# zju3dv/OnePose_Plus_Plus

Hardware: NVIDIA H100
Metric: query images/sec (512x512, 5k 3D pts) (higher is better)
Workload: dtype fp16 hi+lo operand pairs, 3 wgmma MMAs per K-step, fp32 accumulate (fp32-grade)

## Files before the change

### onepose_plus_plus_b200/csrc/opp_common.cuh

```cuda
#pragma once

#include <cuda.h>
#include <cuda_fp16.h>
#include <cuda_runtime.h>
#include <stdint.h>
#include <stdlib.h>

namespace opp {

enum Status : int {
  OPP_OK = 0,
  OPP_ERR_INVALID = 1,
  OPP_ERR_CUDA = 2,
  OPP_ERR_UNSUPPORTED = 3
};

void set_last_error(const char* fmt, ...);

#define OPP_CHECK_CUDA(expr)                                                              \
  do {                                                                                    \
    cudaError_t _e = (expr);                                                              \
    if (_e != cudaSuccess) {                                                              \
      ::opp::set_last_error("%s:%d: %s -> %s", __FILE__, __LINE__, #expr,                 \
                            cudaGetErrorString(_e));                                      \
// ... 201 lines not shown
  return r;
}
__device__ __forceinline__ void cluster_sync_all() {
  asm volatile("barrier.cluster.arrive.aligned;" ::: "memory");
  asm volatile("barrier.cluster.wait.aligned;" ::: "memory");
}

__device__ __forceinline__ uint64_t make_kmajor_sw128_desc(uint32_t smem_addr) {
  uint64_t d = 0;
  d |= static_cast<uint64_t>((smem_addr >> 4) & 0x3FFF);
  d |= static_cast<uint64_t>(1) << 16;
  d |= static_cast<uint64_t>(1024 >> 4) << 32;
  d |= static_cast<uint64_t>(1) << 62;
  return d;
}
__device__ __forceinline__ void wgmma_fence() { asm volatile("wgmma.fence.sync.aligned;" ::: "memory"); }
__device__ __forceinline__ void wgmma_commit() { asm volatile("wgmma.commit_group.sync.aligned;" ::: "memory"); }
template <int N>
__device__ __forceinline__ void wgmma_wait() {
  asm volatile("wgmma.wait_group.sync.aligned %0;" ::"n"(N) : "memory");
}
template <int N>
__device__ __forceinline__ void wgmma_m64nNk16(float (&d)[N / 2], uint64_t a_desc, uint64_t b_desc);
#define OPP_WG_ACC8(i)                                                                              \
  "+f"(d[i]), "+f"(d[i + 1]), "+f"(d[i + 2]), "+f"(d[i + 3]), "+f"(d[i + 4]), "+f"(d[i + 5]),    \
      "+f"(d[i + 6]), "+f"(d[i + 7])
template <>
__device__ __forceinline__ void wgmma_m64nNk16<64>(float (&d)[32], uint64_t a_desc, uint64_t b_desc) {
  asm volatile(
      "{\n\t"
// ... 183 lines not shown
```

### onepose_plus_plus_b200/csrc/opp_gemm.cu

```cuda
#include <cstdarg>
#include <cstdio>
#include <cstdlib>
#include <cstring>
#include <mutex>

#include "../../include/opp_b200.h"
#include "opp_gemm.cuh"

namespace opp {

static thread_local char g_last_error[512] = "";
void set_last_error(const char* fmt, ...) {
  va_list ap;
  va_start(ap, fmt);
  vsnprintf(g_last_error, sizeof(g_last_error), fmt, ap);
  va_end(ap);
}
const char* last_error() { return g_last_error; }

typedef CUresult (*EncodeTiledFn)(CUtensorMap*, CUtensorMapDataType, cuuint32_t, void*,
                                  const cuuint64_t*, const cuuint64_t*, const cuuint32_t*,
                                  const cuuint32_t*, CUtensorMapInterleave, CUtensorMapSwizzle,
                                  CUtensorMapL2promotion, CUtensorMapFloatOOBfill);

// ... 17 lines not shown
    int dev = 0;
    if (cudaGetDevice(&dev) != cudaSuccess) return 132;
    if (cudaDeviceGetAttribute(&n, cudaDevAttrMultiProcessorCount, dev) != cudaSuccess) n = 132;
  }
  return n;
}

static int make_map(CUtensorMap* map, const void* ptr, int rank, const uint64_t* dims,
                    const uint64_t* strides_elems, const uint32_t* box) {
  EncodeTiledFn fn = get_encode_fn();
  if (!fn) {
    set_last_error("cuTensorMapEncodeTiled entry point unavailable (no CUDA driver?)");
    return OPP_ERR_CUDA;
  }
  OPP_REQUIRE((reinterpret_cast<uintptr_t>(ptr) & 15) == 0, "TMA base pointer not 16B aligned");
  cuuint64_t gdim[5], gstr[4];
  cuuint32_t bdim[5], estr[5];
  for (int i = 0; i < rank; ++i) {
    gdim[i] = dims[i];
    bdim[i] = box[i];
    estr[i] = 1;
    OPP_REQUIRE(box[i] >= 1 && box[i] <= 256, "TMA box dim %d = %u out of range", i, box[i]);
  }
  for (int i = 0; i + 1 < rank; ++i) {
    gstr[i] = strides_elems[i] * 2;
    OPP_REQUIRE((gstr[i] & 15) == 0, "TMA stride %d (%llu B) not a multiple of 16", i,
                (unsigned long long)gstr[i]);
  }
  CUresult r = fn(map, CU_TENSOR_MAP_DATA_TYPE_FLOAT16, rank, const_cast<void*>(ptr), gdim, gstr,
                  bdim, estr, CU_TENSOR_MAP_INTERLEAVE_NONE, CU_TENSOR_MAP_SWIZZLE_128B,
                  CU_TENSOR_MAP_L2_PROMOTION_L2_256B, CU_TENSOR_MAP_FLOAT_OOB_FILL_NONE);
  if (r != CUDA_SUCCESS) {
    set_last_error("cuTensorMapEncodeTiled failed with CUresult %d (rank %d dims %llu %llu %llu)",
                   (int)r, rank, (unsigned long long)dims[0], (unsigned long long)dims[1],
                   (unsigned long long)(rank > 2 ? dims[2] : 0));
    return OPP_ERR_CUDA;
  }
  return OPP_OK;
}

static int map_rows(CUtensorMap* map, const void* ptr, long long k, long long rows,
                    long long batches, long long ld, long long batch_stride, int box_rows) {
  uint64_t dims[3] = {(uint64_t)k, (uint64_t)rows, (uint64_t)batches};
  uint64_t str[2] = {(uint64_t)ld, (uint64_t)batch_stride};
  uint32_t box[3] = {(uint32_t)kBlockK, (uint32_t)box_rows, 1};
  return make_map(map, ptr, 3, dims, str, box);
}

static void log_tile_once(int a_mode, const GemmShape& s, const char* epi) {
  static int on = -1;
  if (on < 0) {
    const char* e = getenv("OPP_LOG_TILES");
    on = e ? atoi(e) : 0;
  }
  if (!on) return;
  static std::mutex mu;
  static char seen[256][128];
  static int n_seen = 0;
  char key[128];
  snprintf(key, sizeof(key), "mode %d n %d block_n %d mma_n %d k %d conv_c %d stages %d alias %d cluster %d pair %d",
           a_mode, s.n_total, s.block_n, s.mma_n, s.k_chunks * kBlockK, s.conv_c, s.stages, s.acc_alias,
           s.cluster, s.pair);
  std::lock_guard<std::mutex> lock(mu);
  if (on == 2) {
    fprintf(stderr, "opp gemm tile: %s epi %s\n", key, epi);
    return;
  }
  for (int i = 0; i < n_seen; ++i)
    if (!strcmp(seen[i], key)) return;
  if (n_seen < 256) strcpy(seen[n_seen++], key);
  fprintf(stderr, "opp gemm tile: %s\n", key);
}

template <int A_MODE, class Epi, bool DYN = false>
static int launch(const TensorMaps& maps, GemmShape s, const typename Epi::Params& ep,
                  cudaStream_t stream, const int* rows_dev = nullptr, int rows_mult = 1) {
  {
// ... 3 lines not shown
      dbg = e ? atoi(e) : 0;
    }
    s.debug_skip = dbg;
    static int cap = -1;
    if (cap < 0) {
      const char* e = getenv("OPP_STAGES");
      cap = e ? atoi(e) : 0;
    }
    OPP_REQUIRE(s.mma_n >= EpiMinMmaN<Epi>::value, "GEMM tile width %d below the epilogue's minimum %d",
                s.mma_n, EpiMinMmaN<Epi>::value);
    OPP_REQUIRE(s.mma_n > 0 && gemm_pick_stages<Epi>(s, cap),
                "GEMM tile N=%d (split %d) does not fit in shared memory", s.block_n, s.split);
  }
  const int smem = gemm_smem_bytes<Epi>(s);
  log_tile_once(A_MODE, s, Epi::kName);
  const void* kern;
  if constexpr (DYN) kern = (const void*)gemm_kernel_dyn<A_MODE, Epi>;
  else kern = (const void*)gemm_kernel<A_MODE, Epi>;
  static unsigned long long attr_done = 0;
  int dev = 0;
  OPP_CHECK_CUDA(cudaGetDevice(&dev));
  if (dev < 64 && !((attr_done >> dev) & 1ull)) {
    OPP_CHECK_CUDA(
        cudaFuncSetAttribute(kern, cudaFuncAttributeMaxDynamicSharedMemorySize, 227 * 1024));
    attr_done |= 1ull << dev;
  }
  const long long total = (long long)s.batches * s.msup * s.n_tiles;
  if (total == 0) return OPP_OK;
  const int max_clusters = num_sms() / s.cluster;
  const int n_clusters = (int)(total < max_clusters ? total : max_clusters);
  cudaLaunchConfig_t cfg = {};
  cfg.gridDim = dim3(n_clusters * s.cluster);
  cfg.blockDim = dim3(gemm_threads(Epi::kGroups));
  cfg.dynamicSmemBytes = smem;
  cfg.stream = stream;
  cudaLaunchAttribute attr[2];
  attr[0].id = cudaLaunchAttributeClusterDimension;
  attr[0].val.clusterDim.x = s.cluster;
  attr[0].val.clusterDim.y = 1;
  attr[0].val.clusterDim.z = 1;
// ... 20 lines not shown
  s.cluster = pick_cluster(s.block_n, s.m_tiles);
  s.msup = (s.m_tiles + s.cluster - 1) / s.cluster;
}

static int pick_cluster(int block_n, int m_tiles) {
  static int forced = -1;
  if (forced < 0) {
    const char* e = getenv("OPP_CLUSTER");
    forced = e ? atoi(e) : 0;
  }
  int c = forced > 1 ? forced : 2;
  while (c > 1 && (mma_width_for(block_n) % (8 * c) != 0 || m_tiles < c)) c >>= 1;
  return c;
}

static int pick_block_n(int n) {
  if (n <= 256) return (n + 15) & ~15;
  if (n % 256 == 0) return 256;
  if (n % 128 == 0) return 128;
  return 256;
}

static void split_n_for_latency(GemmShape& s) {
  static int on = -1;
  if (on < 0) {
    const char* e = getenv("OPP_NSPLIT");
    on = e ? atoi(e) : 1;
  }
  if (!on) return;
  const int max_clusters = num_sms() / s.cluster;
// ... 39 lines not shown
                      int min_mma_n = 64) {
  OPP_REQUIRE(a0 && w, "null operand");
  OPP_REQUIRE(k0 > 0 && k0 % 64 == 0 && k1 % 64 == 0, "K (%d,%d) must be multiples of 64", k0,
              k1);
  OPP_REQUIRE(n > 0 && n % n_align == 0, "N=%d must be a multiple of %d", n, n_align);
  OPP_REQUIRE(batches > 0 && rows > 0, "empty GEMM");
  const int planes = split ? 2 : 1;
  memset(&s, 0, sizeof(s));
  s.batches = batches;
  s.rows = (int)rows;
  s.m_tiles = (int)((rows + kBlockM - 1) / kBlockM);
  s.block_n = pick_block_n(n);
  OPP_REQUIRE(s.block_n % 16 == 0 && s.block_n <= 256, "bad block_n %d", s.block_n);
  s.n_tiles = (n + s.block_n - 1) / s.block_n;
  s.n_total = n;
  s.k_chunks_a0 = k0 / 64;
  s.k_chunks = (k0 + k1) / 64;
  s.b_batched = w_batched;
  s.split = split ? 1 : 0;
  s.a0_lo = k0;
  s.a1_lo = k1;
  s.b_lo = k0 + k1;
  s.a0_shared = a0_shared ? 1 : 0;
  const long long ld0 = (long long)planes * k0, ld1 = (long long)planes * k1;
  int rc = map_rows(&maps.a[0], a0, ld0, rows, a0_shared ? 1 : batches, ld0, rows * ld0, kBlockM);
  if (rc) return rc;
  if (k1 > 0) {
    OPP_REQUIRE(a1, "null second A operand");
    rc = map_rows(&maps.a[1], a1, ld1, rows, batches, ld1, rows * ld1, kBlockM);
    if (rc) return rc;
// ... 134 lines not shown
  const int out_w = (in_w + 2 * pad - ksize) / stride + 1;
  TensorMaps maps;
  GemmShape s;
  memset(&s, 0, sizeof(s));
  s.batches = batch;
  s.rows = out_h * out_w;
  s.tile_w = 16;
  s.tile_h = 8;
  s.tiles_x = (out_w + s.tile_w - 1) / s.tile_w;
  s.tiles_y = (out_h + s.tile_h - 1) / s.tile_h;
  s.m_tiles = s.tiles_x * s.tiles_y;
  s.block_n = c_out_pad;
  s.n_tiles = 1;
  s.n_total = c_out_pad;
  s.conv_c = c_in_pad;
  s.conv_cchunks = (c_in_pad + 63) / 64;
  s.k_chunks = ksize * ksize * s.conv_cchunks;
  s.conv_kw = ksize;
  s.conv_pad = pad;
  s.conv_stride = stride;
  s.out_w = out_w;
  s.out_h = out_h;
  s.split = split ? 1 : 0;
  const long long C = (long long)planes * c_in_pad;
  const __half* base = (const __half*)in;
  int rc;
  if (stride == 1) {
    uint64_t dims[5] = {(uint64_t)c_in_pad, (uint64_t)planes, (uint64_t)in_w, (uint64_t)in_h, (uint64_t)batch};
    uint64_t str[4] = {(uint64_t)c_in_pad, (uint64_t)C, (uint64_t)(in_w * C), (uint64_t)((long long)in_h * in_w * C)};
    uint32_t box[5] = {64, 1, (uint32_t)s.tile_w, (uint32_t)s.tile_h, 1};
    rc = make_map(&maps.a[0], base, 5, dims, str, box);
    if (rc) return rc;
    maps.a[1] = maps.a[2] = maps.a[3] = maps.a[0];
  } else {
    for (int py = 0; py < 2; ++py)
      for (int px = 0; px < 2; ++px) {
        uint64_t dims[5] = {(uint64_t)c_in_pad, (uint64_t)planes, (uint64_t)(in_w / 2),
                            (uint64_t)(in_h / 2), (uint64_t)batch};
        uint64_t str[4] = {(uint64_t)c_in_pad, (uint64_t)(2 * C), (uint64_t)(2LL * in_w * C),
                           (uint64_t)((long long)in_h * in_w * C)};
        uint32_t box[5] = {64, 1, (uint32_t)s.tile_w, (uint32_t)s.tile_h, 1};
        rc = make_map(&maps.a[py * 2 + px], base + ((long long)py * in_w + px) * C, 5, dims, str,
                      box);
        if (rc) return rc;
      }
  }
  const long long kplane = (long long)ksize * ksize * c_in_pad;
  s.b_lo = (int)kplane;
  const long long kt = kplane * planes;
  pick_grouping(s);
  split_n_for_latency(s);
  rc = up ? fit_tile<EpiConvUp>(s) : fit_tile<EpiConv>(s);
  if (rc) return rc;
  rc = map_rows(&maps.b, w, kt, c_out_pad, 1, kt, (long long)c_out_pad * kt, s.mma_n / s.cluster);
  if (rc) return rc;
  OPP_REQUIRE(!up || (out_h % 2 == 0 && out_w % 2 == 0 && out_h >= 4 && out_w >= 4),
              "fused upsample-add needs even output dims >= 4 (got %d x %d)", out_h, out_w);
  EpiConvParams ep{(__half*)out, (long long)c_out_pad * planes, split ? c_out_pad : 0, bias,
                     (const __half*)resid, act, slope, (__half*)tok, pe, (const __half*)up,
                     out_h / 2, out_w / 2,
                     up ? (float)(out_h / 2 - 1) / (float)(out_h - 1) : 0.f,
                     up ? (float)(out_w / 2 - 1) / (float)(out_w - 1) : 0.f};
  if (up) return launch<A_CONV, EpiConvUp>(maps, s, ep, (cudaStream_t)stream);
  return launch<A_CONV, EpiConv>(maps, s, ep, (cudaStream_t)stream);
}

int opp_conv_win_pitch(int win) {
  static int pack5 = -1;
  if (pack5 < 0) {
// ... 19 lines not shown
  TensorMaps maps;
  GemmShape s;
  memset(&s, 0, sizeof(s));
  s.batches = 1;
  const int pitch = opp_conv_win_pitch(win);
  s.tile_w = pitch;
  s.tile_h = win;
  s.tiles_x = 128 / (pitch * win);
  s.tiles_y = 1;
  s.rows = matches * pitch * win;
  s.m_tiles = (matches + s.tiles_x - 1) / s.tiles_x;
  s.block_n = c_out_pad;
  s.n_tiles = 1;
  s.n_total = c_out_pad;
  s.conv_c = c_in_pad;
  s.conv_cchunks = (c_in_pad + 63) / 64;
  s.k_chunks = 9 * s.conv_cchunks;
  s.conv_kw = 3;
  s.conv_pad = 1;
  s.conv_stride = 1;
  s.out_w = pitch;
  s.out_h = win;
  s.split = split ? 1 : 0;
  const long long C = (long long)planes * c_in_pad;
  int rc;
  {
    const uint64_t iw = j_ids ? in_w : 8, ih = j_ids ? in_h : win + 2, ib = j_ids ? batch : matches;
    uint64_t dims[5] = {(uint64_t)c_in_pad, (uint64_t)planes, iw, ih, ib};
    uint64_t str[4] = {(uint64_t)c_in_pad, (uint64_t)C, (uint64_t)(iw * C), (uint64_t)(ih * iw * C)};
    uint32_t box[5] = {64, 1, (uint32_t)pitch, (uint32_t)win, 1};
    rc = make_map(&maps.a[0], in, 5, dims, str, box);
    if (rc) return rc;
    maps.a[1] = maps.a[2] = maps.a[3] = maps.a[0];
  }
  const long long kplane = 9LL * c_in_pad;
  s.b_lo = (int)kplane;
  const long long kt = kplane * planes;
  pick_grouping(s);
  rc = fit_tile<EpiWin>(s);
  if (rc) return rc;
  rc = map_rows(&maps.b, w, kt, c_out_pad, 1, kt, (long long)c_out_pad * kt, s.mma_n / s.cluster);
  if (rc) return rc;
  EpiWin::Params ep{(__half*)out, (long long)c_out_pad * planes, split ? c_out_pad : 0, bias, act, slope,
                    b_ids, j_ids, wc, stride, org, in_h, in_w};
  if (count) return launch<A_WIN, EpiWin, true>(maps, s, ep, (cudaStream_t)stream, count, pitch * win);
  return launch<A_WIN, EpiWin>(maps, s, ep, (cudaStream_t)stream);
}

int opp_sim_lse(const void* a, const void* b, float* part_m, float* part_s, int batches, int rows,
                int cols, int k, float scale, int split, opp_stream_t stream) {
  TensorMaps maps;
  GemmShape s;
  int rc = setup_rows(maps, s, a, k, nullptr, 0, b, 1, batches, rows, cols, split, 1);
  if (rc) return rc;
  EpiLse::Params ep{part_m, part_s, scale};
  return launch<A_ROWS, EpiLse>(maps, s, ep, (cudaStream_t)stream);
// ... 72 lines not shown
```

### onepose_plus_plus_b200/csrc/opp_gemm.cuh

```cuda
#pragma once

#include <type_traits>

#include "opp_common.cuh"

#ifndef OPP_CONV_GROUPS
#define OPP_CONV_GROUPS 2
#endif

namespace opp {

constexpr int kBlockM = 128;
constexpr int kBlockK = 64;
constexpr int kABytes = kBlockM * kBlockK * 2;
constexpr int kMaxStages = 8;
constexpr int kEpiParamBytes = 4096;
constexpr int kMaxEpiWarps = 8;
constexpr int gemm_threads(int groups) { return 128 + 128 * groups; }
constexpr int kProducerRegs = 40;
constexpr int kMmaRegs = 232;
static_assert(128 * kProducerRegs + 256 * kMmaRegs <= 65536, "register file of one SM");
constexpr int kMmaWidths[] = {64, 128, 208, 256};
constexpr int mma_width_for(int block_n) {
  for (int w : kMmaWidths)
    if (w >= block_n) return w;
  return 0;
}

enum AMode : int { A_ROWS = 0, A_CONV = 1, A_WIN = 2 };

struct TensorMaps {
  CUtensorMap a[4];
  CUtensorMap b;
};

struct GemmShape {
  int batches;
  int rows;
  int m_tiles;
  int n_tiles;
  int n_total;
  int block_n;
  int mma_n;
  int k_chunks;
  int stages;
  int b_batched;
  int cluster;
  int msup;
  int pair;
  int acc_alias;
  int debug_skip;
  int split;
  int b_lo;
  int k_chunks_a0;
  int a0_lo, a1_lo;
  int a0_shared;
  int conv_cchunks;
  int conv_c;
  int conv_kw;
// ... 1184 lines not shown
}

template <int N, int KS>
__device__ __forceinline__ void mma_k_steps(float (&d)[N / 2], bool split, uint64_t a_hi, uint64_t a_lo,
                                            uint64_t b_hi, uint64_t b_lo) {
#pragma unroll
  for (int k = 0; k < KS; ++k) wgmma_m64nNk16<N>(d, a_hi + 2 * k, b_hi + 2 * k);
  if (split) {
#pragma unroll
    for (int k = 0; k < KS; ++k) wgmma_m64nNk16<N>(d, a_hi + 2 * k, b_lo + 2 * k);
#pragma unroll
    for (int k = 0; k < KS; ++k) wgmma_m64nNk16<N>(d, a_lo + 2 * k, b_hi + 2 * k);
  }
}

template <int A_MODE, class Epi>
__device__ __forceinline__ void gemm_body(const TensorMaps& maps, const GemmShape& s,
                                          const typename Epi::Params& ep) {
  static_assert(Epi::kGroups == 2, "each of the two MMA warpgroups is one epilogue group");
  extern __shared__ uint8_t smem_raw[];
  uint8_t* smem = reinterpret_cast<uint8_t*>(
      (reinterpret_cast<uintptr_t>(smem_raw) + 1023) & ~static_cast<uintptr_t>(1023));
  const int planes = s.split ? 2 : 1;
  const bool nsc = s.pair == 2;
  const int b_bytes = s.mma_n * kBlockK * 2;
  const int a_stage = kABytes * planes;
  const int b_stage = b_bytes * planes;
  const int ring = s.stages * (a_stage + b_stage);
  uint8_t* smem_a = smem;
  uint8_t* smem_b = smem + s.stages * a_stage;
  constexpr bool kAccTile = !EpiFromRegs<Epi>::value;
  uint8_t* smem_acc = s.acc_alias ? smem : smem + ring;
  float* epi_smem = reinterpret_cast<float*>(smem + ring + (kAccTile && !s.acc_alias ? gemm_acc_bytes(s.mma_n) : 0));
  uint64_t* bars = reinterpret_cast<uint64_t*>(reinterpret_cast<uint8_t*>(epi_smem) +
                                               epi_smem_bytes<Epi>());
  uint64_t* full = bars;
  uint64_t* empty = bars + kMaxStages;
  uint64_t* accfree = bars + 2 * kMaxStages;

  constexpr int kProducerWarp = 4 * Epi::kGroups;
  const int warp = threadIdx.x >> 5;
  const int lane = threadIdx.x & 31;
  const int csize = nsc ? 1 : s.cluster;
  const int prank = s.cluster > 1 ? (int)cluster_ctarank() : 0;
  const int crank = nsc ? 0 : prank;
  const int nrank = nsc ? prank : 0;
  const uint16_t cmask = (uint16_t)((1u << csize) - 1u);
  const int cluster_id = blockIdx.x / s.cluster;
  const int n_clusters = gridDim.x / s.cluster;
  const int tiles_per_batch = s.msup * s.n_tiles;
  const int total_tiles = s.batches * tiles_per_batch;

  if (warp == kProducerWarp && lane == 0) {
    tma_prefetch_desc(&maps.a[0]);
    tma_prefetch_desc(&maps.b);
  }
  if (warp == 0 && lane == 0) {
    for (int i = 0; i < s.stages; ++i) {
      mbar_init(&full[i], 1);
      mbar_init(&empty[i], 2 * csize);
    }
    mbar_init(accfree, 4 * Epi::kGroups * csize);
    if constexpr (EpiExtraSmem<Epi>::value > 0) {
      uint64_t* xbar = reinterpret_cast<uint64_t*>(reinterpret_cast<uint8_t*>(epi_smem) + epi_smem_bytes<Epi>() -
                                                   EpiExtraSmem<Epi>::value + 2 * 128 * 8);
      mbar_init(&xbar[0], Epi::kExchangeArrivals);
      mbar_init(&xbar[1], Epi::kExchangeArrivals);
    }
    fence_mbar_init();
  }
  if (s.cluster > 1) cluster_sync_all(); else __syncthreads();
  pdl_sync();

  if (warp >= kProducerWarp) {
    setmaxnreg_dec<kProducerRegs>();
    if (warp == kProducerWarp) {
      int stage = 0;
      uint32_t phase = 0;
      const bool skip_b = (s.debug_skip & 1) != 0, skip_a = (s.debug_skip & 2) != 0;
      const int a_tx = A_MODE == A_WIN ? s.tiles_x * s.tile_w * s.tile_h * (kBlockK * 2) * planes : a_stage;
      const uint32_t tx_bytes = (skip_a ? 0 : a_tx) + (skip_b ? 0 : b_stage);
      int it = 0;
      for (int t = cluster_id; t < total_tiles; t += n_clusters, ++it) {
        if (s.acc_alias && it > 0) mbar_wait(accfree, (uint32_t)((it - 1) & 1));
        const int b = t / tiles_per_batch;
        const int r = t - b * tiles_per_batch;
        const int msi = r / s.n_tiles;
        const int n_tile = nsc ? nrank : r - msi * s.n_tiles;
        const int m_tile = msi * csize + crank;
        int ox0 = 0, oy0 = 0;
        if (A_MODE == A_CONV) {
          const int ty = m_tile / s.tiles_x;
          oy0 = ty * s.tile_h;
          ox0 = (m_tile - ty * s.tiles_x) * s.tile_w;
        }
// ... 6 lines not shown
          for (int wi = 0; wi < 5; ++wi) {
            int m = m_tile * s.tiles_x + wi;
            m = m < cnt ? m : cnt - 1;
            win_z[wi] = m;
            if (ep.j_ids) {
              const int j = (int)ep.j_ids[m];
              const int cy = j / ep.wc;
              win_z[wi] = (int)ep.b_ids[m];
              win_x[wi] = ep.stride * (j - cy * ep.wc) + ep.org - s.conv_pad;
              win_y[wi] = ep.stride * cy + ep.org - s.conv_pad;
            }
          }
        }
        int cc = 0, ky = 0, kx = 0, kb_tap = 0;
        for (int chunk = 0; chunk < s.k_chunks; ++chunk) {
          mbar_wait(&empty[stage], phase ^ 1);
          uint8_t* sa = smem_a + stage * a_stage;
          uint8_t* sb = smem_b + stage * b_stage;
          int kb;
          if (A_MODE == A_ROWS) {
            const bool first = chunk < s.k_chunks_a0;
            const int kc = (first ? chunk : chunk - s.k_chunks_a0) * kBlockK;
            const CUtensorMap* am = first ? &maps.a[0] : &maps.a[1];
            const int lo = first ? s.a0_lo : s.a1_lo;
            const int ba = (first && s.a0_shared) ? 0 : b;
            kb = chunk * kBlockK;
            if (elect_one()) {
              mbar_expect_tx(&full[stage], tx_bytes);
              if (!skip_a) {
                tma_load_3d(am, &full[stage], sa, kc, m_tile * kBlockM, ba);
                if (s.split) tma_load_3d(am, &full[stage], sa + kABytes, kc + lo, m_tile * kBlockM, ba);
              }
            }
          } else if constexpr (A_MODE == A_WIN) {
            kb = kb_tap + cc * kBlockK;
            const int wbytes = s.tile_w * s.tile_h * (kBlockK * 2);
#pragma unroll
            for (int wi = 0; wi < 5; ++wi) {
              if (wi >= s.tiles_x) break;
              const int bx = win_x[wi] + kx, by = win_y[wi] + ky, bz = win_z[wi];
              if (elect_one()) {
                if (wi == 0) mbar_expect_tx(&full[stage], tx_bytes);
                if (!skip_a) {
                  tma_load_5d(&maps.a[0], &full[stage], sa + wi * wbytes, cc * kBlockK, 0, bx, by, bz);
                  if (s.split)
                    tma_load_5d(&maps.a[0], &full[stage], sa + kABytes + wi * wbytes, cc * kBlockK, 1, bx, by, bz);
                }
              }
            }
            if (++cc == s.conv_cchunks) {
              cc = 0;
              kb_tap += s.conv_c;
              if (++kx == s.conv_kw) {
                kx = 0;
                ++ky;
              }
            }
          } else {
            int dy = ky - s.conv_pad, dx = kx - s.conv_pad, mi = 0;
            if (s.conv_stride == 2) {
              const int py = dy & 1, px = dx & 1;
              dy = (dy - py) >> 1;
              dx = (dx - px) >> 1;
              mi = py * 2 + px;
            }
            kb = kb_tap + cc * kBlockK;
            if (elect_one()) {
              mbar_expect_tx(&full[stage], tx_bytes);
              if (!skip_a) {
                tma_load_5d(&maps.a[mi], &full[stage], sa, cc * kBlockK, 0, ox0 + dx, oy0 + dy, b);
                if (s.split)
                  tma_load_5d(&maps.a[mi], &full[stage], sa + kABytes, cc * kBlockK, 1, ox0 + dx, oy0 + dy, b);
              }
            }
            if (++cc == s.conv_cchunks) {
              cc = 0;
              kb_tap += s.conv_c;
              if (++kx == s.conv_kw) {
                kx = 0;
                ++ky;
              }
            }
          }
          if (!skip_b && elect_one()) {
            if (csize == 1) {
              tma_load_3d(&maps.b, &full[stage], sb, kb, nrow0, bb);
              if (s.split) tma_load_3d(&maps.b, &full[stage], sb + b_bytes, s.b_lo + kb, nrow0, bb);
            } else {
              const int slice = s.mma_n / csize;
              const int soff = crank * slice * (kBlockK * 2);
              const int nrow = nrow0 + crank * slice;
              tma_load_3d_mc(&maps.b, &full[stage], sb + soff, kb, nrow, bb, cmask);
              if (s.split)
                tma_load_3d_mc(&maps.b, &full[stage], sb + b_bytes + soff, s.b_lo + kb, nrow, bb, cmask);
            }
          }
          __syncwarp();
          if (++stage == s.stages) {
            stage = 0;
            phase ^= 1;
          }
        }
      }
    }
  } else {
    setmaxnreg_inc<kMmaRegs>();
    const int g = warp >> 2;
    const int q = warp & 3;
    EpiCtx c;
    c.etid = q * 32 + lane;
    c.q = q;
    c.a_mode = A_MODE;
    c.group = g;
    c.col_first = 32 * g;
    c.col_step = 32 * Epi::kGroups;
    c.smem = epi_smem + g * (kEpiParamBytes / 8);
    c.wstage = reinterpret_cast<uint8_t*>(epi_smem) + kEpiParamBytes + warp * EpiWarpStage<Epi>::value;
    c.extra = reinterpret_cast<uint8_t*>(epi_smem) + epi_smem_bytes<Epi>() - EpiExtraSmem<Epi>::value;
    c.smem_s = smem_u32(c.smem);
    c.wstage_s = smem_u32(c.wstage);
    const uint64_t desc_tmpl = make_kmajor_sw128_desc(0);
    const uint32_t sa0 = ((smem_u32(smem_a) >> 4) & 0x3FFF) + g * ((64 * 128) >> 4);
    const uint32_t sb0 = (smem_u32(smem_b) >> 4) & 0x3FFF;
    const uint32_t a_step = (uint32_t)a_stage >> 4, b_step = (uint32_t)b_stage >> 4;
    const uint32_t a_lo_off = kABytes >> 4, b_lo_off = (uint32_t)b_bytes >> 4;
    const bool split = s.split != 0;
    const bool is_signal = q == 0 && lane == 0;
    const uint32_t pitch = (uint32_t)(s.mma_n + kAccPad);
    const uint32_t acc_w = smem_u32(smem_acc) >> 2;
    const uint32_t r0 = 64 * g + 16 * q + (lane >> 2), c0 = 2 * (lane & 3);
    auto release = [&](int st) {
      if (is_signal) {
        if (csize == 1) mbar_arrive(&empty[st]);
        else
          for (int r = 0; r < csize; ++r) mbar_arrive_cluster(&empty[st], (uint32_t)r);
      }
    };
// ... 34 lines not shown
          int rdummy;
          if (epi_row_at(s, c, (int)r0 + 8 * h, c.sgrow[h], rdummy)) c.svalid |= 1u << h;
        }
      }
      c.acc = acc_w + (uint32_t)(q * 32 + lane) * pitch;
      Epi::prefetch(ep, s, c);

      auto mma_tile = [&](auto n_c, auto tail_c) {
        constexpr int N = decltype(n_c)::value;
        constexpr int TAIL = decltype(tail_c)::value;
        float d[N / 2];
#pragma unroll
        for (int i = 0; i < N / 2; ++i) d[i] = 0.f;
        wgmma_fence_acc(d);
        int prev = -1;
        auto chunk_step = [&](auto ks_c, auto& acc) {
          const uint64_t a_hi = desc_tmpl | sa, b_hi = desc_tmpl | sb;
          const uint64_t a_lo = desc_tmpl | (sa + a_lo_off), b_lo = desc_tmpl | (sb + b_lo_off);
          mbar_wait_hot(&full[stage], phase);
          wgmma_fence();
          mma_k_steps<N, decltype(ks_c)::value>(acc, split, a_hi, a_lo, b_hi, b_lo);
          wgmma_commit();
          wgmma_fence_acc(acc);
          if (prev >= 0) {
            wgmma_wait<1>();
            release(prev);
          }
          prev = stage;
          sa += a_step;
          sb += b_step;
          if (++stage == s.stages) {
            stage = 0;
            phase ^= 1;
            sa = sa0;
            sb = sb0;
          }
        };
        if constexpr (TAIL == 0) {
          for (int chunk = 0; chunk < s.k_chunks; ++chunk) chunk_step(std::integral_constant<int, 4>{}, d);
        } else {
          const int taps = s.k_chunks / s.conv_cchunks;
          for (int tap = 0; tap < taps; ++tap) {
            for (int cc = 1; cc < s.conv_cchunks; ++cc) chunk_step(std::integral_constant<int, 4>{}, d);
            chunk_step(std::integral_constant<int, TAIL>{}, d);
          }
        }
        wgmma_wait<0>();
        wgmma_fence_acc(d);
        if (prev >= 0) release(prev);

        if constexpr (!kAccTile) {
          if (!(s.debug_skip & 4)) Epi::template run_frag<N>(ep, s, c, d);
        } else {
          named_bar_sync(4, 256);
#pragma unroll
          for (int i = 0; i < N / 8; ++i) {
            const uint32_t col = 8 * i + c0;
            sts64f((acc_w + r0 * pitch + col) * 4, d[4 * i], d[4 * i + 1]);
            sts64f((acc_w + (r0 + 8) * pitch + col) * 4, d[4 * i + 2], d[4 * i + 3]);
// ... 27 lines not shown
          __syncwarp();
          if (lane == 0) {
            if (csize == 1) mbar_arrive(accfree);
            else
              for (int r2 = 0; r2 < csize; ++r2) mbar_arrive_cluster(accfree, (uint32_t)r2);
          }
        }
      }
    }
  }

  pdl_done();
  if (s.cluster > 1) cluster_sync_all(); else __syncthreads();
}

template <int A_MODE, class Epi>
__global__ void __launch_bounds__(gemm_threads(Epi::kGroups), 1)
gemm_kernel(const __grid_constant__ TensorMaps maps, const GemmShape s, const typename Epi::Params ep) {
  gemm_body<A_MODE, Epi>(maps, s, ep);
}

template <int A_MODE, class Epi>
__global__ void __launch_bounds__(gemm_threads(Epi::kGroups), 1)
gemm_kernel_dyn(const __grid_constant__ TensorMaps maps, const GemmShape s_in,
                const typename Epi::Params ep, const int* rows_dev, int rows_mult) {
  GemmShape s = s_in;
  pdl_wait();
  const int r = *rows_dev * rows_mult;
  s.rows = r < s_in.rows ? r : s_in.rows;
  const int tile_rows = A_MODE == A_WIN ? s_in.tiles_x * s_in.tile_w * s_in.tile_h : kBlockM;
  s.m_tiles = (s.rows + tile_rows - 1) / tile_rows;
  s.msup = (s.m_tiles + s_in.cluster - 1) / s_in.cluster;
  gemm_body<A_MODE, Epi>(maps, s, ep);
}

inline int gemm_stage_bytes(int mma_n, int split) {
  return (kABytes + mma_n * kBlockK * 2) * (split ? 2 : 1);
}
template <class Epi>
inline int gemm_smem_bytes(const GemmShape& s) {
  const bool acc_tile = !EpiFromRegs<Epi>::value && !s.acc_alias;
  return s.stages * gemm_stage_bytes(s.mma_n, s.split) + (acc_tile ? gemm_acc_bytes(s.mma_n) : 0) +
         epi_smem_bytes<Epi>() + (2 * kMaxStages + 2) * 8 + 16 + 1024;
}
constexpr int kSmemLimit = 227 * 1024;
template <class Epi>
inline bool gemm_pick_stages(GemmShape& s, int cap = 0) {
  const int avail = kSmemLimit - epi_smem_bytes<Epi>() - 2048;
  const int sb = gemm_stage_bytes(s.mma_n, s.split);
  const int ab = EpiFromRegs<Epi>::value ? 0 : gemm_acc_bytes(s.mma_n);
  int st = (avail - ab) / sb;
  s.acc_alias = ab > 0 && st < 2;
  if (s.acc_alias) st = avail / sb;
  if (st > kMaxStages) st = kMaxStages;
  if (st > s.k_chunks * 2 && s.k_chunks * 2 >= 2) st = s.k_chunks * 2;
  if (cap > 1 && st > cap) st = cap;
  if (st < 2) st = 2;
  if (s.acc_alias && st * sb < ab) st = (ab + sb - 1) / sb;
  s.stages = st;
  return st <= kMaxStages && gemm_smem_bytes<Epi>(s) <= kSmemLimit;
}

}
```

Measured before the change: 432.0.

## Split conv K-chunks into 32-wide ring slots with 64B swizzle for wide 3x3 layers

Adds a BK=32 variant of the GEMM kernel. Each 64-channel K chunk is split into two half-width pipeline slots using 64B-swizzled TMA boxes and matching wgmma descriptors. The variant is chosen by default for 3x3 convs with more than 128 output channels. The aim is a finer-grained producer/consumer pipeline, with more, smaller stages in flight for the same shared memory, to cut stall time on wide conv layers. In exchange it doubles the mbarrier traffic and TMA issue count per chunk, and it adds a tail-chunk path that issues a zero-width MMA step.

```diff
diff --git a/onepose_plus_plus_b200/csrc/opp_common.cuh b/onepose_plus_plus_b200/csrc/opp_common.cuh
--- a/onepose_plus_plus_b200/csrc/opp_common.cuh
+++ b/onepose_plus_plus_b200/csrc/opp_common.cuh
@@ -239,6 +239,14 @@
   d |= static_cast<uint64_t>(1) << 62;
   return d;
 }
+__device__ __forceinline__ uint64_t make_kmajor_sw64_desc(uint32_t smem_addr) {
+  uint64_t d = 0;
+  d |= static_cast<uint64_t>((smem_addr >> 4) & 0x3FFF);
+  d |= static_cast<uint64_t>(1) << 16;
+  d |= static_cast<uint64_t>(512 >> 4) << 32;
+  d |= static_cast<uint64_t>(2) << 62;
+  return d;
+}
 __device__ __forceinline__ void wgmma_fence() { asm volatile("wgmma.fence.sync.aligned;" ::: "memory"); }
 __device__ __forceinline__ void wgmma_commit() { asm volatile("wgmma.commit_group.sync.aligned;" ::: "memory"); }
 template <int N>
diff --git a/onepose_plus_plus_b200/csrc/opp_gemm.cu b/onepose_plus_plus_b200/csrc/opp_gemm.cu
--- a/onepose_plus_plus_b200/csrc/opp_gemm.cu
+++ b/onepose_plus_plus_b200/csrc/opp_gemm.cu
@@ -55,6 +55,7 @@
     return OPP_ERR_CUDA;
   }
   OPP_REQUIRE((reinterpret_cast<uintptr_t>(ptr) & 15) == 0, "TMA base pointer not 16B aligned");
+  OPP_REQUIRE(box[0] == 64 || box[0] == 32, "TMA inner box %u is not one swizzle row", box[0]);
   cuuint64_t gdim[5], gstr[4];
   cuuint32_t bdim[5], estr[5];
   for (int i = 0; i < rank; ++i) {
@@ -69,7 +70,8 @@
                 (unsigned long long)gstr[i]);
   }
   CUresult r = fn(map, CU_TENSOR_MAP_DATA_TYPE_FLOAT16, rank, const_cast<void*>(ptr), gdim, gstr,
-                  bdim, estr, CU_TENSOR_MAP_INTERLEAVE_NONE, CU_TENSOR_MAP_SWIZZLE_128B,
+                  bdim, estr, CU_TENSOR_MAP_INTERLEAVE_NONE,
+                  box[0] == 32 ? CU_TENSOR_MAP_SWIZZLE_64B : CU_TENSOR_MAP_SWIZZLE_128B,
                   CU_TENSOR_MAP_L2_PROMOTION_L2_256B, CU_TENSOR_MAP_FLOAT_OOB_FILL_NONE);
   if (r != CUDA_SUCCESS) {
     set_last_error("cuTensorMapEncodeTiled failed with CUresult %d (rank %d dims %llu %llu %llu)",
@@ -81,10 +83,10 @@
 }
 
 static int map_rows(CUtensorMap* map, const void* ptr, long long k, long long rows,
-                    long long batches, long long ld, long long batch_stride, int box_rows) {
+                    long long batches, long long ld, long long batch_stride, int box_rows, int bk = kBlockK) {
   uint64_t dims[3] = {(uint64_t)k, (uint64_t)rows, (uint64_t)batches};
   uint64_t str[2] = {(uint64_t)ld, (uint64_t)batch_stride};
-  uint32_t box[3] = {(uint32_t)kBlockK, (uint32_t)box_rows, 1};
+  uint32_t box[3] = {(uint32_t)bk, (uint32_t)box_rows, 1};
   return make_map(map, ptr, 3, dims, str, box);
 }
 
@@ -99,9 +101,9 @@
   static char seen[256][128];
   static int n_seen = 0;
   char key[128];
-  snprintf(key, sizeof(key), "mode %d n %d block_n %d mma_n %d k %d conv_c %d stages %d alias %d cluster %d pair %d",
+  snprintf(key, sizeof(key), "mode %d n %d block_n %d mma_n %d k %d conv_c %d stages %d alias %d cluster %d pair %d bk %d",
            a_mode, s.n_total, s.block_n, s.mma_n, s.k_chunks * kBlockK, s.conv_c, s.stages, s.acc_alias,
-           s.cluster, s.pair);
+           s.cluster, s.pair, s.bk);
   std::lock_guard<std::mutex> lock(mu);
   if (on == 2) {
     fprintf(stderr, "opp gemm tile: %s epi %s\n", key, epi);
@@ -135,16 +137,25 @@
   }
   const int smem = gemm_smem_bytes<Epi>(s);
   log_tile_once(A_MODE, s, Epi::kName);
+  OPP_REQUIRE(s.bk == kBlockK || (s.bk == 32 && A_MODE != A_ROWS), "ring slot width %d not compiled for mode %d",
+              s.bk, A_MODE);
   const void* kern;
   if constexpr (DYN) kern = (const void*)gemm_kernel_dyn<A_MODE, Epi>;
   else kern = (const void*)gemm_kernel<A_MODE, Epi>;
-  static unsigned long long attr_done = 0;
+  if constexpr (A_MODE != A_ROWS) {
+    if (s.bk == 32) {
+      if constexpr (DYN) kern = (const void*)gemm_kernel_dyn<A_MODE, Epi, 32>;
+      else kern = (const void*)gemm_kernel<A_MODE, Epi, 32>;
+    }
+  }
+  static unsigned long long attr_done[2] = {0, 0};
+  unsigned long long& done = attr_done[s.bk == 32];
   int dev = 0;
   OPP_CHECK_CUDA(cudaGetDevice(&dev));
-  if (dev < 64 && !((attr_done >> dev) & 1ull)) {
+  if (dev < 64 && !((done >> dev) & 1ull)) {
     OPP_CHECK_CUDA(
         cudaFuncSetAttribute(kern, cudaFuncAttributeMaxDynamicSharedMemorySize, 227 * 1024));
-    attr_done |= 1ull << dev;
+    done |= 1ull << dev;
   }
   const long long total = (long long)s.batches * s.msup * s.n_tiles;
   if (total == 0) return OPP_OK;
@@ -195,6 +206,16 @@
   return c;
 }
 
+static int conv_chunk_k(int ksize, int c_out_pad) {
+  static int forced = -1;
+  if (forced < 0) {
+    const char* e = getenv("OPP_CONV_BK");
+    forced = e ? atoi(e) : 0;
+  }
+  if (forced == 32 || forced == 64) return forced;
+  return ksize == 3 && c_out_pad > 128 ? 32 : 64;
+}
+
 static int pick_block_n(int n) {
   if (n <= 256) return (n + 15) & ~15;
   if (n % 256 == 0) return 256;
@@ -264,6 +285,7 @@
   OPP_REQUIRE(s.block_n % 16 == 0 && s.block_n <= 256, "bad block_n %d", s.block_n);
   s.n_tiles = (n + s.block_n - 1) / s.block_n;
   s.n_total = n;
+  s.bk = kBlockK;
   s.k_chunks_a0 = k0 / 64;
   s.k_chunks = (k0 + k1) / 64;
   s.b_batched = w_batched;
@@ -428,6 +450,7 @@
   s.n_tiles = 1;
   s.n_total = c_out_pad;
   s.conv_c = c_in_pad;
+  s.bk = conv_chunk_k(ksize, c_out_pad);
   s.conv_cchunks = (c_in_pad + 63) / 64;
   s.k_chunks = ksize * ksize * s.conv_cchunks;
   s.conv_kw = ksize;
@@ -442,7 +465,7 @@
   if (stride == 1) {
     uint64_t dims[5] = {(uint64_t)c_in_pad, (uint64_t)planes, (uint64_t)in_w, (uint64_t)in_h, (uint64_t)batch};
     uint64_t str[4] = {(uint64_t)c_in_pad, (uint64_t)C, (uint64_t)(in_w * C), (uint64_t)((long long)in_h * in_w * C)};
-    uint32_t box[5] = {64, 1, (uint32_t)s.tile_w, (uint32_t)s.tile_h, 1};
+    uint32_t box[5] = {(uint32_t)s.bk, 1, (uint32_t)s.tile_w, (uint32_t)s.tile_h, 1};
     rc = make_map(&maps.a[0], base, 5, dims, str, box);
     if (rc) return rc;
     maps.a[1] = maps.a[2] = maps.a[3] = maps.a[0];
@@ -453,7 +476,7 @@
                             (uint64_t)(in_h / 2), (uint64_t)batch};
         uint64_t str[4] = {(uint64_t)c_in_pad, (uint64_t)(2 * C), (uint64_t)(2LL * in_w * C),
                            (uint64_t)((long long)in_h * in_w * C)};
-        uint32_t box[5] = {64, 1, (uint32_t)s.tile_w, (uint32_t)s.tile_h, 1};
+        uint32_t box[5] = {(uint32_t)s.bk, 1, (uint32_t)s.tile_w, (uint32_t)s.tile_h, 1};
         rc = make_map(&maps.a[py * 2 + px], base + ((long long)py * in_w + px) * C, 5, dims, str,
                       box);
         if (rc) return rc;
@@ -466,7 +489,7 @@
   split_n_for_latency(s);
   rc = up ? fit_tile<EpiConvUp>(s) : fit_tile<EpiConv>(s);
   if (rc) return rc;
-  rc = map_rows(&maps.b, w, kt, c_out_pad, 1, kt, (long long)c_out_pad * kt, s.mma_n / s.cluster);
+  rc = map_rows(&maps.b, w, kt, c_out_pad, 1, kt, (long long)c_out_pad * kt, s.mma_n / s.cluster, s.bk);
   if (rc) return rc;
   OPP_REQUIRE(!up || (out_h % 2 == 0 && out_w % 2 == 0 && out_h >= 4 && out_w >= 4),
               "fused upsample-add needs even output dims >= 4 (got %d x %d)", out_h, out_w);
@@ -516,6 +539,8 @@
   s.n_tiles = 1;
   s.n_total = c_out_pad;
   s.conv_c = c_in_pad;
+  s.bk = conv_chunk_k(3, c_out_pad);
+  OPP_REQUIRE(pitch == 8 || s.bk == 64, "OPP_WIN5_PACK needs 64-wide ring slots (layer has %d)", s.bk);
   s.conv_cchunks = (c_in_pad + 63) / 64;
   s.k_chunks = 9 * s.conv_cchunks;
   s.conv_kw = 3;
@@ -530,7 +555,7 @@
     const uint64_t iw = j_ids ? in_w : 8, ih = j_ids ? in_h : win + 2, ib = j_ids ? batch : matches;
     uint64_t dims[5] = {(uint64_t)c_in_pad, (uint64_t)planes, iw, ih, ib};
     uint64_t str[4] = {(uint64_t)c_in_pad, (uint64_t)C, (uint64_t)(iw * C), (uint64_t)(ih * iw * C)};
-    uint32_t box[5] = {64, 1, (uint32_t)pitch, (uint32_t)win, 1};
+    uint32_t box[5] = {(uint32_t)s.bk, 1, (uint32_t)pitch, (uint32_t)win, 1};
     rc = make_map(&maps.a[0], in, 5, dims, str, box);
     if (rc) return rc;
     maps.a[1] = maps.a[2] = maps.a[3] = maps.a[0];
@@ -541,7 +566,7 @@
   pick_grouping(s);
   rc = fit_tile<EpiWin>(s);
   if (rc) return rc;
-  rc = map_rows(&maps.b, w, kt, c_out_pad, 1, kt, (long long)c_out_pad * kt, s.mma_n / s.cluster);
+  rc = map_rows(&maps.b, w, kt, c_out_pad, 1, kt, (long long)c_out_pad * kt, s.mma_n / s.cluster, s.bk);
   if (rc) return rc;
   EpiWin::Params ep{(__half*)out, (long long)c_out_pad * planes, split ? c_out_pad : 0, bias, act, slope,
                     b_ids, j_ids, wc, stride, org, in_h, in_w};
diff --git a/onepose_plus_plus_b200/csrc/opp_gemm.cuh b/onepose_plus_plus_b200/csrc/opp_gemm.cuh
--- a/onepose_plus_plus_b200/csrc/opp_gemm.cuh
+++ b/onepose_plus_plus_b200/csrc/opp_gemm.cuh
@@ -12,7 +12,7 @@
 
 constexpr int kBlockM = 128;
 constexpr int kBlockK = 64;
-constexpr int kABytes = kBlockM * kBlockK * 2;
+__host__ __device__ constexpr int gemm_a_bytes(int bk) { return kBlockM * bk * 2; }
 constexpr int kMaxStages = 8;
 constexpr int kEpiParamBytes = 4096;
 constexpr int kMaxEpiWarps = 8;
@@ -43,6 +43,7 @@
   int block_n;
   int mma_n;
   int k_chunks;
+  int bk;
   int stages;
   int b_batched;
   int cluster;
@@ -1257,21 +1258,25 @@
   }
 }
 
-template <int A_MODE, class Epi>
+template <int A_MODE, class Epi, int BK>
 __device__ __forceinline__ void gemm_body(const TensorMaps& maps, const GemmShape& s,
                                           const typename Epi::Params& ep) {
   static_assert(Epi::kGroups == 2, "each of the two MMA warpgroups is one epilogue group");
+  static_assert(BK == 64 || BK == 32, "K chunk of one 128B- or 64B-swizzle row");
+  constexpr int kABytes = gemm_a_bytes(BK);
   extern __shared__ uint8_t smem_raw[];
   uint8_t* smem = reinterpret_cast<uint8_t*>(
       (reinterpret_cast<uintptr_t>(smem_raw) + 1023) & ~static_cast<uintptr_t>(1023));
   const int planes = s.split ? 2 : 1;
   const bool nsc = s.pair == 2;
-  const int b_bytes = s.mma_n * kBlockK * 2;
+  constexpr int kParts = kBlockK / BK;
+  const int slots = s.stages * kParts;
+  const int b_bytes = s.mma_n * BK * 2;
   const int a_stage = kABytes * planes;
   const int b_stage = b_bytes * planes;
-  const int ring = s.stages * (a_stage + b_stage);
+  const int ring = slots * (a_stage + b_stage);
   uint8_t* smem_a = smem;
-  uint8_t* smem_b = smem + s.stages * a_stage;
+  uint8_t* smem_b = smem + slots * a_stage;
   constexpr bool kAccTile = !EpiFromRegs<Epi>::value;
   uint8_t* smem_acc = s.acc_alias ? smem : smem + ring;
   float* epi_smem = reinterpret_cast<float*>(smem + ring + (kAccTile && !s.acc_alias ? gemm_acc_bytes(s.mma_n) : 0));
@@ -1299,7 +1304,7 @@
     tma_prefetch_desc(&maps.b);
   }
   if (warp == 0 && lane == 0) {
-    for (int i = 0; i < s.stages; ++i) {
+    for (int i = 0; i < slots; ++i) {
       mbar_init(&full[i], 1);
       mbar_init(&empty[i], 2 * csize);
     }
@@ -1321,7 +1326,7 @@
       int stage = 0;
       uint32_t phase = 0;
       const bool skip_b = (s.debug_skip & 1) != 0, skip_a = (s.debug_skip & 2) != 0;
-      const int a_tx = A_MODE == A_WIN ? s.tiles_x * s.tile_w * s.tile_h * (kBlockK * 2) * planes : a_stage;
+      const int a_tx = A_MODE == A_WIN ? s.tiles_x * s.tile_w * s.tile_h * (BK * 2) * planes : a_stage;
       const uint32_t tx_bytes = (skip_a ? 0 : a_tx) + (skip_b ? 0 : b_stage);
       int it = 0;
       for (int t = cluster_id; t < total_tiles; t += n_clusters, ++it) {
@@ -1358,91 +1363,86 @@
         }
         int cc = 0, ky = 0, kx = 0, kb_tap = 0;
         for (int chunk = 0; chunk < s.k_chunks; ++chunk) {
-          mbar_wait(&empty[stage], phase ^ 1);
-          uint8_t* sa = smem_a + stage * a_stage;
-          uint8_t* sb = smem_b + stage * b_stage;
-          int kb;
-          if (A_MODE == A_ROWS) {
-            const bool first = chunk < s.k_chunks_a0;
-            const int kc = (first ? chunk : chunk - s.k_chunks_a0) * kBlockK;
-            const CUtensorMap* am = first ? &maps.a[0] : &maps.a[1];
-            const int lo = first ? s.a0_lo : s.a1_lo;
-            const int ba = (first && s.a0_shared) ? 0 : b;
-            kb = chunk * kBlockK;
-            if (elect_one()) {
-              mbar_expect_tx(&full[stage], tx_bytes);
-              if (!skip_a) {
-                tma_load_3d(am, &full[stage], sa, kc, m_tile * kBlockM, ba);
-                if (s.split) tma_load_3d(am, &full[stage], sa + kABytes, kc + lo, m_tile * kBlockM, ba);
+          const bool first = A_MODE == A_ROWS && chunk < s.k_chunks_a0;
+          const int ka = A_MODE == A_ROWS ? (first ? chunk : chunk - s.k_chunks_a0) * kBlockK : cc * kBlockK;
+          const int kb = A_MODE == A_ROWS ? chunk * kBlockK : kb_tap + ka;
+#pragma unroll
+          for (int part = 0; part < kParts; ++part) {
+            const int kp = part * BK;
+            mbar_wait(&empty[stage], phase ^ 1);
+            uint8_t* sa = smem_a + stage * a_stage;
+            uint8_t* sb = smem_b + stage * b_stage;
+            {
+              if constexpr (A_MODE == A_ROWS) {
+                const CUtensorMap* am = first ? &maps.a[0] : &maps.a[1];
+                const int lo = first ? s.a0_lo : s.a1_lo;
+                const int ba = (first && s.a0_shared) ? 0 : b;
+                if (elect_one()) {
+                  mbar_expect_tx(&full[stage], tx_bytes);
+                  if (!skip_a) {
+                    tma_load_3d(am, &full[stage], sa, ka + kp, m_tile * kBlockM, ba);
+                    if (s.split) tma_load_3d(am, &full[stage], sa + kABytes, ka + kp + lo, m_tile * kBlockM, ba);
+                  }
+                }
+              } else if constexpr (A_MODE == A_WIN) {
+                const int wbytes = s.tile_w * s.tile_h * (BK * 2);
+#pragma unroll
+                for (int wi = 0; wi < 5; ++wi) {
+                  if (wi >= s.tiles_x) break;
+                  const int bx = win_x[wi] + kx, by = win_y[wi] + ky, bz = win_z[wi];
+                  if (elect_one()) {
+                    if (wi == 0) mbar_expect_tx(&full[stage], tx_bytes);
+                    if (!skip_a) {
+                      tma_load_5d(&maps.a[0], &full[stage], sa + wi * wbytes, ka + kp, 0, bx, by, bz);
+                      if (s.split)
+                        tma_load_5d(&maps.a[0], &full[stage], sa + kABytes + wi * wbytes, ka + kp, 1, bx, by, bz);
+                    }
+                  }
+                }
+              } else {
+                int dy = ky - s.conv_pad, dx = kx - s.conv_pad, mi = 0;
+                if (s.conv_stride == 2) {
+                  const int py = dy & 1, px = dx & 1;
+                  dy = (dy - py) >> 1;
+                  dx = (dx - px) >> 1;
+                  mi = py * 2 + px;
+                }
+                const CUtensorMap* am = &maps.a[mi];
+                if (elect_one()) {
+                  mbar_expect_tx(&full[stage], tx_bytes);
+                  if (!skip_a) {
+                    tma_load_5d(am, &full[stage], sa, ka + kp, 0, ox0 + dx, oy0 + dy, b);
+                    if (s.split) tma_load_5d(am, &full[stage], sa + kABytes, ka + kp, 1, ox0 + dx, oy0 + dy, b);
+                  }
+                }
               }
-            }
-          } else if constexpr (A_MODE == A_WIN) {
-            kb = kb_tap + cc * kBlockK;
-            const int wbytes = s.tile_w * s.tile_h * (kBlockK * 2);
-#pragma unroll
-            for (int wi = 0; wi < 5; ++wi) {
-              if (wi >= s.tiles_x) break;
-              const int bx = win_x[wi] + kx, by = win_y[wi] + ky, bz = win_z[wi];
-              if (elect_one()) {
-                if (wi == 0) mbar_expect_tx(&full[stage], tx_bytes);
-                if (!skip_a) {
-                  tma_load_5d(&maps.a[0], &full[stage], sa + wi * wbytes, cc * kBlockK, 0, bx, by, bz);
+              if (!skip_b && elect_one()) {
+                if (csize == 1) {
+                  tma_load_3d(&maps.b, &full[stage], sb, kb + kp, nrow0, bb);
+                  if (s.split) tma_load_3d(&maps.b, &full[stage], sb + b_bytes, s.b_lo + kb + kp, nrow0, bb);
+                } else {
+                  const int slice = s.mma_n / csize;
+                  const int soff = crank * slice * (BK * 2);
+                  const int nrow = nrow0 + crank * slice;
+                  tma_load_3d_mc(&maps.b, &full[stage], sb + soff, kb + kp, nrow, bb, cmask);
                   if (s.split)
-                    tma_load_5d(&maps.a[0], &full[stage], sa + kABytes + wi * wbytes, cc * kBlockK, 1, bx, by, bz);
+                    tma_load_3d_mc(&maps.b, &full[stage], sb + b_bytes + soff, s.b_lo + kb + kp, nrow, bb, cmask);
                 }
               }
             }
-            if (++cc == s.conv_cchunks) {
-              cc = 0;
-              kb_tap += s.conv_c;
-              if (++kx == s.conv_kw) {
-                kx = 0;
-                ++ky;
-              }
-            }
-          } else {
-            int dy = ky - s.conv_pad, dx = kx - s.conv_pad, mi = 0;
-            if (s.conv_stride == 2) {
-              const int py = dy & 1, px = dx & 1;
-              dy = (dy - py) >> 1;
-              dx = (dx - px) >> 1;
-              mi = py * 2 + px;
-            }
-            kb = kb_tap + cc * kBlockK;
-            if (elect_one()) {
-              mbar_expect_tx(&full[stage], tx_bytes);
-              if (!skip_a) {
-                tma_load_5d(&maps.a[mi], &full[stage], sa, cc * kBlockK, 0, ox0 + dx, oy0 + dy, b);
-                if (s.split)
-                  tma_load_5d(&maps.a[mi], &full[stage], sa + kABytes, cc * kBlockK, 1, ox0 + dx, oy0 + dy, b);
-              }
-            }
-            if (++cc == s.conv_cchunks) {
-              cc = 0;
-              kb_tap += s.conv_c;
-              if (++kx == s.conv_kw) {
-                kx = 0;
-                ++ky;
-              }
+            __syncwarp();
+            if (++stage == slots) {
+              stage = 0;
+              phase ^= 1;
             }
           }
-          if (!skip_b && elect_one()) {
-            if (csize == 1) {
-              tma_load_3d(&maps.b, &full[stage], sb, kb, nrow0, bb);
-              if (s.split) tma_load_3d(&maps.b, &full[stage], sb + b_bytes, s.b_lo + kb, nrow0, bb);
-            } else {
-              const int slice = s.mma_n / csize;
-              const int soff = crank * slice * (kBlockK * 2);
-              const int nrow = nrow0 + crank * slice;
-              tma_load_3d_mc(&maps.b, &full[stage], sb + soff, kb, nrow, bb, cmask);
-              if (s.split)
-                tma_load_3d_mc(&maps.b, &full[stage], sb + b_bytes + soff, s.b_lo + kb, nrow, bb, cmask);
+          if (A_MODE != A_ROWS && ++cc == s.conv_cchunks) {
+            cc = 0;
+            kb_tap += s.conv_c;
+            if (++kx == s.conv_kw) {
+              kx = 0;
+              ++ky;
             }
-          }
-          __syncwarp();
-          if (++stage == s.stages) {
-            stage = 0;
-            phase ^= 1;
           }
         }
       }
@@ -1463,8 +1463,8 @@
     c.extra = reinterpret_cast<uint8_t*>(epi_smem) + epi_smem_bytes<Epi>() - EpiExtraSmem<Epi>::value;
     c.smem_s = smem_u32(c.smem);
     c.wstage_s = smem_u32(c.wstage);
-    const uint64_t desc_tmpl = make_kmajor_sw128_desc(0);
-    const uint32_t sa0 = ((smem_u32(smem_a) >> 4) & 0x3FFF) + g * ((64 * 128) >> 4);
+    const uint64_t desc_tmpl = BK == 64 ? make_kmajor_sw128_desc(0) : make_kmajor_sw64_desc(0);
+    const uint32_t sa0 = ((smem_u32(smem_a) >> 4) & 0x3FFF) + g * ((64 * BK * 2) >> 4);
     const uint32_t sb0 = (smem_u32(smem_b) >> 4) & 0x3FFF;
     const uint32_t a_step = (uint32_t)a_stage >> 4, b_step = (uint32_t)b_stage >> 4;
     const uint32_t a_lo_off = kABytes >> 4, b_lo_off = (uint32_t)b_bytes >> 4;
@@ -1529,6 +1529,7 @@
         for (int i = 0; i < N / 2; ++i) d[i] = 0.f;
         wgmma_fence_acc(d);
         int prev = -1;
+        static_assert(TAIL * 16 <= BK, "a tail chunk's channels lie in its first slot");
         auto chunk_step = [&](auto ks_c, auto& acc) {
           const uint64_t a_hi = desc_tmpl | sa, b_hi = desc_tmpl | sb;
           const uint64_t a_lo = desc_tmpl | (sa + a_lo_off), b_lo = desc_tmpl | (sb + b_lo_off);
@@ -1544,20 +1545,28 @@
           prev = stage;
           sa += a_step;
           sb += b_step;
-          if (++stage == s.stages) {
+          if (++stage == slots) {
             stage = 0;
             phase ^= 1;
             sa = sa0;
             sb = sb0;
           }
         };
+        auto full_chunk = [&]() {
+#pragma unroll
+          for (int part = 0; part < kParts; ++part) chunk_step(std::integral_constant<int, BK / 16>{}, d);
+        };
+        auto tail_chunk = [&]() {
+          chunk_step(std::integral_constant<int, TAIL>{}, d);
+          if constexpr (kParts == 2) chunk_step(std::integral_constant<int, 0>{}, d);
+        };
         if constexpr (TAIL == 0) {
-          for (int chunk = 0; chunk < s.k_chunks; ++chunk) chunk_step(std::integral_constant<int, 4>{}, d);
+          for (int chunk = 0; chunk < s.k_chunks; ++chunk) full_chunk();
         } else {
           const int taps = s.k_chunks / s.conv_cchunks;
           for (int tap = 0; tap < taps; ++tap) {
-            for (int cc = 1; cc < s.conv_cchunks; ++cc) chunk_step(std::integral_constant<int, 4>{}, d);
-            chunk_step(std::integral_constant<int, TAIL>{}, d);
+            for (int cc = 1; cc < s.conv_cchunks; ++cc) full_chunk();
+            tail_chunk();
           }
         }
         wgmma_wait<0>();
@@ -1615,13 +1624,13 @@
   if (s.cluster > 1) cluster_sync_all(); else __syncthreads();
 }
 
-template <int A_MODE, class Epi>
+template <int A_MODE, class Epi, int BK = kBlockK>
 __global__ void __launch_bounds__(gemm_threads(Epi::kGroups), 1)
 gemm_kernel(const __grid_constant__ TensorMaps maps, const GemmShape s, const typename Epi::Params ep) {
-  gemm_body<A_MODE, Epi>(maps, s, ep);
-}
-
-template <int A_MODE, class Epi>
+  gemm_body<A_MODE, Epi, BK>(maps, s, ep);
+}
+
+template <int A_MODE, class Epi, int BK = kBlockK>
 __global__ void __launch_bounds__(gemm_threads(Epi::kGroups), 1)
 gemm_kernel_dyn(const __grid_constant__ TensorMaps maps, const GemmShape s_in,
                 const typename Epi::Params ep, const int* rows_dev, int rows_mult) {
@@ -1632,11 +1641,11 @@
   const int tile_rows = A_MODE == A_WIN ? s_in.tiles_x * s_in.tile_w * s_in.tile_h : kBlockM;
   s.m_tiles = (s.rows + tile_rows - 1) / tile_rows;
   s.msup = (s.m_tiles + s_in.cluster - 1) / s_in.cluster;
-  gemm_body<A_MODE, Epi>(maps, s, ep);
+  gemm_body<A_MODE, Epi, BK>(maps, s, ep);
 }
 
 inline int gemm_stage_bytes(int mma_n, int split) {
-  return (kABytes + mma_n * kBlockK * 2) * (split ? 2 : 1);
+  return (gemm_a_bytes(kBlockK) + mma_n * kBlockK * 2) * (split ? 2 : 1);
 }
 template <class Epi>
 inline int gemm_smem_bytes(const GemmShape& s) {
@@ -1649,17 +1658,18 @@
 inline bool gemm_pick_stages(GemmShape& s, int cap = 0) {
   const int avail = kSmemLimit - epi_smem_bytes<Epi>() - 2048;
   const int sb = gemm_stage_bytes(s.mma_n, s.split);
+  const int max_st = kMaxStages * s.bk / kBlockK;
   const int ab = EpiFromRegs<Epi>::value ? 0 : gemm_acc_bytes(s.mma_n);
   int st = (avail - ab) / sb;
   s.acc_alias = ab > 0 && st < 2;
   if (s.acc_alias) st = avail / sb;
-  if (st > kMaxStages) st = kMaxStages;
+  if (st > max_st) st = max_st;
   if (st > s.k_chunks * 2 && s.k_chunks * 2 >= 2) st = s.k_chunks * 2;
   if (cap > 1 && st > cap) st = cap;
   if (st < 2) st = 2;
   if (s.acc_alias && st * sb < ab) st = (ab + sb - 1) / sb;
   s.stages = st;
-  return st <= kMaxStages && gemm_smem_bytes<Epi>(s) <= kSmemLimit;
-}
-
-}
+  return st <= max_st && gemm_smem_bytes<Epi>(s) <= kSmemLimit;
+}
+
+}
```

Result: faster. 477.5 (median of 6 runs) (+10.5%).
